# pyxploiter/HandMvNet

Measured on AMD Instinct MI355X. Metric: samples/sec (BxV frames) eval_fps.py, 8-view 256x256; 21-kpt L2 vs reference, higher is better.
Workload: dtype f32; 1 GPU; BASELINE configs[2]: B=32/GPU x V=8 x 256x256, resnet50_paper backbone, d=524, cross_attn x5, GCN decoder; global_batch=32, views=8, frame=256, parallelism=sample-shard x1

## Files before the change

handmvnet_amd/csrc/conv_stream.hip:

```cpp
#include <cstdio>
#include <cstdlib>
#include <type_traits>
#include <utility>

#include "kernels.h"

namespace hmv {

typedef float sf32x16 __attribute__((ext_vector_type(16)));
typedef float sf32x4 __attribute__((ext_vector_type(4)));
typedef _Float16 sf16x8 __attribute__((ext_vector_type(8)));

#define HMV_SGLDS16(gptr, lptr)                                                                             \
    __builtin_amdgcn_global_load_lds((const __attribute__((address_space(1))) void *)(gptr),                \
                                     (__attribute__((address_space(3))) void *)(lptr), 16, 0, 0)

template <int N>
__device__ __forceinline__ void wait_vm() {
    static_assert(N >= 0 && N < 64, "vmcnt is a 6-bit field");
    asm volatile("s_waitcnt vmcnt(%0)" ::"n"(N) : "memory");
}
template <typename F, int... I>
__device__ __forceinline__ void static_for_impl(F &&f, std::integer_sequence<int, I...>) {
    (f(std::integral_constant<int, I>{}), ...);
}
template <int N, typename F>
__device__ __forceinline__ void static_for(F &&f) {
    static_for_impl(static_cast<F &&>(f), std::make_integer_sequence<int, N>{});
}

constexpr int sched_r(int RB, int RS, int j) { return RS ? RS : (j == 0 ? RB : 0); }
constexpr int sched_ops(int NP, int PA, int RB, int RS, int OS, int slot) { return slot < NP ? PA + sched_r(RB, RS, slot) : OS; }
constexpr int sched_after_piece(int NP, int D, int PA, int RB, int RS, int OS, int j) {
    const int T0 = 8, g = T0 * NP + j - D, tq = g / NP, jq = g - tq * NP;
    int n = sched_r(RB, RS, jq);
    for (int s = tq * (NP + 1) + jq + 1; s < T0 * (NP + 1) + j; ++s) n += sched_ops(NP, PA, RB, RS, OS, s % (NP + 1));
    return n;
}
constexpr int sched_after_residual(int NP, int PA, int RB, int RS, int OS) {
    const int T0 = 8, last = RS ? NP - 1 : 0;
    int n = 0;
    for (int s = (T0 - 1) * (NP + 1) + last + 1; s < T0 * (NP + 1) + NP; ++s) n += sched_ops(NP, PA, RB, RS, OS, s % (NP + 1));
    return n;
}
static_assert(sched_after_piece(4, 3, 1, 8, 0, 8, 0) == 10 && sched_after_piece(4, 3, 1, 8, 0, 8, 1) == 18 && sched_after_piece(4, 3, 1, 8, 0, 8, 2) == 18 &&
              sched_after_piece(4, 3, 1, 8, 0, 8, 3) == 10 && sched_after_residual(4, 1, 8, 0, 8) == 23, "the step-0 schedule of four pieces, counted by hand");
static_assert(sched_after_piece(4, 3, 1, 8, 2, 8, 0) == 2 + 3 + 3 + 8 && sched_after_residual(4, 1, 8, 2, 8) == 8 + 4 * 3, "the spread K = 256 schedule");

template <int TM, int TN, int MW, int NW, int NP, int NSLOT, bool HAS_RES, bool SPREAD = false, bool DUAL = false, int N2 = 0>
__global__ __launch_bounds__(64 * MW *NW, (MW * NW) / 4) void conv_stream_f16(const ConvParams p) {
    constexpr int NWV = MW * NW, NT = 64 * NWV;
    constexpr int BM = 32 * TM * MW, BN = 32 * TN * NW;
    constexpr int D = NSLOT - 1;
    constexpr int PA = BM * 8 / NT;
    constexpr int NB2 = N2 / 32;
    constexpr int TM2 = N2 ? (BM / 32) * NB2 / NWV : 0;
    constexpr int K2Q = BN / 16;
    static_assert(N2 == 0 || (N2 % 32 == 0 && TN == 2 && TM2 >= 1 && NWV % NB2 == 0 && (BM / 32) == (NWV / NB2) * TM2),
                  "chain: a wave's 64 output channels are one pixel piece of the second reduction; whole blocks per wave");
    constexpr int RB = HAS_RES ? TM * TN * 2 : 0, OS = TM * TN * 2 + 2 * TM2;
    constexpr int RS = (SPREAD && HAS_RES) ? RB / NP : 0;
    static_assert(!SPREAD || RB % NP == 0, "spread schedule: whole residual DMAs per step");
    constexpr int ZW = TM * TN * 2 * 1024;
    constexpr int NFAKE = (D + NP - 1) / NP;
    static_assert(NT == 512 && BM % 64 == 0 && PA >= 1, "eight waves; whole DMA passes per piece");
    static_assert((NSLOT & (NSLOT - 1)) == 0 && NSLOT >= 2, "a power of two");
    extern __shared__ __attribute__((aligned(16))) char ssm[];
    _Float16 *sA = reinterpret_cast<_Float16 *>(ssm);
    char *zones = ssm + NSLOT * BM * 128;

    const int tid = threadIdx.x, lane = tid & 63;
    const int wave = __builtin_amdgcn_readfirstlane(tid >> 6);
    const int l31 = lane & 31, kh = lane >> 5;
    const int mw = wave / NW, nw = wave - mw * NW;
    const int zi = N2 ? nw * MW + mw : wave;
    static_assert(N2 == 0 || !HAS_RES || ZW == TM * 32 * 128, "chain: a landing zone is the wave's region of the tile image");

    const int nsl = p.ntiles;
    const int loc = (int)blockIdx.x >> 3, per_xcd = 32 / nsl;
    const int slice = loc % nsl, stream = ((int)blockIdx.x & 7) * per_xcd + loc / nsl, nstreams = 8 * per_xcd;
    const int ntl = p.mtiles > stream ? (p.mtiles - stream + nstreams - 1) / nstreams : 0;
    if (ntl == 0) return;
    const int n0 = slice * BN + nw * TN * 32;

    const _Float16 *zero16 = reinterpret_cast<const _Float16 *>(p.zero);
    _Float16 *trash = reinterpret_cast<_Float16 *>(const_cast<float *>(p.zero) + 64 + 4 * lane);
    const _Float16 *Ain = reinterpret_cast<const _Float16 *>(p.in);
    const _Float16 *Rin = reinterpret_cast<const _Float16 *>(p.res);
    _Float16 *Out = reinterpret_cast<_Float16 *>(p.out);

    const int wl31 = (l31 & 0x13) | ((l31 & 4) << 1) | ((l31 & 8) >> 1);
    sf16x8 wreg[TN][NP * 4];
    {
        const _Float16 *wb = reinterpret_cast<const _Float16 *>(p.wgt) + (size_t)(n0 + wl31) * p.ldw + 8 * kh;
#pragma unroll
        for (int b = 0; b < TN; ++b)
#pragma unroll
            for (int Q = 0; Q < NP * 4; ++Q) wreg[b][Q] = *reinterpret_cast<const sf16x8 *>(wb + (size_t)(32 * b) * p.ldw + 16 * Q);
    }
    const int ob2 = N2 ? wave % (N2 ? NB2 : 1) : 0, pg2 = N2 ? wave / (N2 ? NB2 : 1) : 0;
    sf16x8 w2reg[N2 ? K2Q : 1];
    if constexpr (N2 > 0) {
        const _Float16 *wb2 = reinterpret_cast<const _Float16 *>(p.nx_wgt) + (size_t)(32 * ob2 + wl31) * p.nx_ldw + 8 * kh;
#pragma unroll
        for (int Q = 0; Q < K2Q; ++Q) w2reg[Q] = *reinterpret_cast<const sf16x8 *>(wb2 + 16 * Q);
    }
    asm volatile("s_waitcnt vmcnt(0)" ::: "memory");

    const int arow = tid >> 3, kqs = (tid & 7) ^ ((tid >> 4) & 7);
    const int fsw = (l31 >> 1) & 7;

    size_t off2[DUAL ? PA : 1] = {};
    auto issue_A = [&](int G) {
        const int tt = G >= 0 ? G / NP : -1, jj = G >= 0 ? G - tt * NP : 0, slot = G & (NSLOT - 1);
        const int mt = stream + tt * nstreams;
#pragma unroll
        for (int i = 0; i < PA; ++i) {
            const int m = mt * BM + i * 64 + arow;
            const bool ok = tt >= 0 && tt < ntl && m < p.M;
            const _Float16 *src = zero16;
            if constexpr (DUAL) {
                if (jj * 64 == p.ksplit) {
                    const int hw = p.Ho * p.Wo, n = m / hw, rem = m - n * hw, ho = rem / p.Wo, wo = rem - ho * p.Wo;
                    off2[i] = ((size_t)(n * p.H2 + ho * p.stride2) * p.W2 + wo * p.stride2) * p.lda2 + 8 * kqs;
                }
                if (ok && jj * 64 >= p.ksplit) {
                    src = reinterpret_cast<const _Float16 *>(p.in2) + off2[i] + (jj * 64 - p.ksplit);
                } else if (ok) {
                    src = Ain + (size_t)m * p.lda + jj * 64 + 8 * kqs;
                }
// ... 122 lines not shown
                                            (unsigned)((nw * BM + (mw * TM + a) * 32 + l31) * 128 + (((4 * b + 2 * j + kh) ^ fsw) * 16));
                        asm volatile("ds_write_b128 %0, %1" ::"v"(ya), "v"(hv[a][b][j]) : "memory");
                    }
            }
            asm volatile("s_waitcnt lgkmcnt(0)\n\ts_barrier" ::: "memory");
            const __attribute__((address_space(4))) float *bq =
                (const __attribute__((address_space(4))) float *)(p.nx_bias + __builtin_amdgcn_readfirstlane(32 * ob2)) + bz;
            sf32x16 acc2[TM2];
#pragma unroll
            for (int e = 0; e < 16; ++e) {
                const int c = 16 * (e >> 3) + (e & 7);
                const float v0 = bq[c], v1 = bq[c + 8];
                const float v = kh ? v1 : v0;
#pragma unroll
                for (int a = 0; a < TM2; ++a) acc2[a][e] = v;
            }
            const unsigned yr = (unsigned)(size_t)(__attribute__((address_space(3))) char *)yt + (unsigned)((pg2 * TM2 * 32 + l31) * 128);
            constexpr int G = 4 / TM2, NG = K2Q / G;
            static_assert(K2Q % G == 0 && G * TM2 == 4, "four fragment reads per group");
            sf16x8 px[2][G][TM2];
#define HMV_CHAIN_READ_GROUP(g)                                                                                                     \
    _Pragma("unroll") for (int i = 0; i < G; ++i) _Pragma("unroll") for (int a = 0; a < TM2; ++a) {                                \
        const int Q = (g) * G + i;                                                                                                  \
        const unsigned ad = yr + (unsigned)(((Q >> 2) * BM + a * 32) * 128) + (unsigned)((((2 * (Q & 3) + kh) ^ fsw)) * 16);        \
        asm volatile("ds_read_b128 %0, %1" : "=v"(px[(g) & 1][i][a]) : "v"(ad) : "memory");                                         \
    }
            HMV_CHAIN_READ_GROUP(0)
#pragma unroll
            for (int g = 0; g < NG; ++g) {
                sf16x8(&pg)[G][TM2] = px[g & 1];
                if (g + 1 < NG) {
                    HMV_CHAIN_READ_GROUP(g + 1)
                    if constexpr (TM2 == 1) asm volatile("s_waitcnt lgkmcnt(4)" : "+v"(pg[0][0]), "+v"(pg[1][0]), "+v"(pg[2][0]), "+v"(pg[3][0]) :: "memory");
                    else asm volatile("s_waitcnt lgkmcnt(4)" : "+v"(pg[0][0]), "+v"(pg[0][1]), "+v"(pg[1][0]), "+v"(pg[1][1]) :: "memory");
                } else {
                    if constexpr (TM2 == 1) asm volatile("s_waitcnt lgkmcnt(0)" : "+v"(pg[0][0]), "+v"(pg[1][0]), "+v"(pg[2][0]), "+v"(pg[3][0]) :: "memory");
                    else asm volatile("s_waitcnt lgkmcnt(0)" : "+v"(pg[0][0]), "+v"(pg[0][1]), "+v"(pg[1][0]), "+v"(pg[1][1]) :: "memory");
                }
#pragma unroll
                for (int i = 0; i < G; ++i)
#pragma unroll
                    for (int a = 0; a < TM2; ++a) acc2[a] = __builtin_amdgcn_mfma_f32_32x32x16_f16(w2reg[g * G + i], pg[i][a], acc2[a], 0, 0, 0);
            }
#undef HMV_CHAIN_READ_GROUP
            const float lo2 = (p.nx_act == ACT_RELU) ? 0.f : -INFINITY;
            _Float16 *Out2 = reinterpret_cast<_Float16 *>(p.nx_out);
#pragma unroll
            for (int a = 0; a < TM2; ++a) {
                const int m = mt * BM + (pg2 * TM2 + a) * 32 + l31;
                _Float16 *orow = Out2 + (size_t)m * p.nx_ldc + 32 * ob2 + 8 * kh;
#pragma unroll
                for (int j = 0; j < 2; ++j) {
                    const sf16x8 r = {0, 0, 0, 0, 0, 0, 0, 0};
                    sf16x8 h2;
#pragma unroll
                    for (int u = 0; u < 8; ++u) h2[u] = (_Float16)fmaxf(acc2[a][8 * j + u] * p.acc_scale + (float)r[u], lo2);
                    _Float16 *dst = m < p.M ? orow + 16 * j : trash;
                    asm volatile("global_store_dwordx4 %0, %1, off\n\ts_nop 1" ::"v"(dst), "v"(h2) : "memory");
                }
            }
        } else {
#pragma unroll
        for (int a = 0; a < TM; ++a) {
            const int m = mt * BM + (mw * TM + a) * 32 + l31;
            _Float16 *orow = Out + (size_t)m * p.ldc + n0 + 8 * kh;
#pragma unroll
            for (int b = 0; b < TN; ++b)
#pragma unroll
                for (int j = 0; j < 2; ++j) {
                    sf16x8 r = {0, 0, 0, 0, 0, 0, 0, 0};
                    if constexpr (HAS_RES) r = *reinterpret_cast<const sf16x8 *>(z + ((a * TN + b) * 2 + j) * 1024);
                    sf16x8 hv;
#pragma unroll
                    for (int u = 0; u < 8; ++u) hv[u] = (_Float16)fmaxf(acc[a][b][8 * j + u] * p.acc_scale + (float)r[u], lo);
                    _Float16 *dst = m < p.M ? orow + 32 * b + 16 * j : trash;
                    asm volatile("global_store_dwordx4 %0, %1, off\n\ts_nop 1" ::"v"(dst), "v"(hv) : "memory");
                }
        }
        }
    }
    asm volatile("s_waitcnt vmcnt(0) lgkmcnt(0)" ::: "memory");
}

template <int TM, int TN, int MW, int NW, int NP, int NSLOT, bool HAS_RES, bool DUAL = false, bool HALF = false>
__global__ __launch_bounds__(64 * MW *NW, 2) void conv_stream_f32(const ConvParams p) {
    constexpr int NWV = MW * NW, NT = 64 * NWV;
    constexpr int BM = 32 * TM * MW, BN = 32 * TN * NW;
    constexpr int D = NSLOT - 1;
    constexpr int PA = BM * 8 / NT;
    constexpr int RB = HAS_RES ? TM * TN * 4 : 0, OS = TM * TN * 4, RS = 0;
    constexpr int ZW = TM * TN * 4 * 1024;
    constexpr int NFAKE = (D + NP - 1) / NP;
    constexpr int RPP = NT / 8;
    static_assert((NT == 512 || (HALF && NT == 256)) && BM % RPP == 0 && PA >= 1 && (!HALF || (HAS_RES && !DUAL)), "whole DMA passes per piece");
    static_assert((NSLOT & (NSLOT - 1)) == 0 && NSLOT >= 2, "a power of two");
    extern __shared__ __attribute__((aligned(16))) char ssm[];
    float *sA = reinterpret_cast<float *>(ssm);
    char *zones = ssm + NSLOT * BM * 128;

    const int tid = threadIdx.x, lane = tid & 63;
    const int wave = __builtin_amdgcn_readfirstlane(tid >> 6);
    const int l31 = lane & 31, kh = lane >> 5;
    const int mw = wave / NW, nw = wave - mw * NW;
    const int nsl = p.ntiles;
    const int loc = (int)blockIdx.x >> 3, per_xcd = ((int)gridDim.x >> 3) / nsl;
    const int slice = loc % nsl, stream = ((int)blockIdx.x & 7) * per_xcd + loc / nsl, nstreams = 8 * per_xcd;
    const int ntl = p.mtiles > stream ? (p.mtiles - stream + nstreams - 1) / nstreams : 0;
    if (ntl == 0) return;
    const int n0 = slice * BN + nw * TN * 32;

    const float *zero32 = p.zero;
    float *trash = const_cast<float *>(p.zero) + 64 + 4 * lane;
    const float *Ain = reinterpret_cast<const float *>(p.in);
    const float *Rin = reinterpret_cast<const float *>(p.res);
    float *Out = reinterpret_cast<float *>(p.out);

    sf32x4 wreg[TN][NP * 4], bias[TN][4];
    {
        const float *wb = reinterpret_cast<const float *>(p.wgt) + (size_t)(n0 + l31) * p.ldw + 4 * kh;
#pragma unroll
        for (int b = 0; b < TN; ++b) {
#pragma unroll
            for (int Q = 0; Q < NP * 4; ++Q) wreg[b][Q] = *reinterpret_cast<const sf32x4 *>(wb + (size_t)(32 * b) * p.ldw + 8 * Q);
#pragma unroll
            for (int g = 0; g < 4; ++g) bias[b][g] = *reinterpret_cast<const sf32x4 *>(p.bias + n0 + 32 * b + 8 * g + 4 * kh);
        }
    }
    asm volatile("s_waitcnt vmcnt(0)" ::: "memory");

    const int arow = tid >> 3, kqs = (tid & 7) ^ ((tid >> 4) & 7);
    const int fsw = (l31 >> 1) & 7;
    auto issue_A = [&](int G) {
        const int tt = G >= 0 ? G / NP : -1, jj = G >= 0 ? G - tt * NP : 0, slot = G & (NSLOT - 1);
        const int mt = stream + tt * nstreams;
#pragma unroll
        for (int i = 0; i < PA; ++i) {
            const int m = mt * BM + i * RPP + arow;
            const bool ok = tt >= 0 && tt < ntl && m < p.M;
            const float *src = zero32;
            if constexpr (DUAL) {
                if (ok && jj * 32 >= p.ksplit) {
                    const int hw = p.Ho * p.Wo, n = m / hw, rem = m - n * hw, ho = rem / p.Wo, wo = rem - ho * p.Wo;
                    src = reinterpret_cast<const float *>(p.in2) + ((size_t)(n * p.H2 + ho * p.stride2) * p.W2 + wo * p.stride2) * p.lda2 +
                          (jj * 32 - p.ksplit) + 4 * kqs;
                } else if (ok) {
                    src = Ain + (size_t)m * p.lda + jj * 32 + 4 * kqs;
                }
            } else if (ok) {
                src = Ain + (size_t)m * p.lda + jj * 32 + 4 * kqs;
            }
            asm volatile("" : "+v"(src));
            HMV_SGLDS16(src, sA + ((slot * BM + i * RPP + wave * 8) * 32));
        }
    };
    auto issue_R = [&](int tt) {
        if constexpr (HAS_RES) {
            const int mt = stream + tt * nstreams;
            char *z = zones + ((HALF ? 0 : (tt & 1)) * NWV + wave) * ZW;
#pragma unroll
            for (int idx = 0; idx < RB; ++idx) {
                const int a = idx / (4 * TN), b = (idx / 4) % TN, g = idx & 3;
                const int m = mt * BM + (mw * TM + a) * 32 + l31;
                const bool ok = tt >= 0 && tt < ntl && m < p.M;
                const float *src = ok ? Rin + (size_t)m * p.ldr + n0 + 32 * b + 8 * g + 4 * kh : zero32;
                asm volatile("" : "+v"(src));
                HMV_SGLDS16(src, z + idx * 1024);
            }
        }
    };
#pragma unroll
    for (int ft = -NFAKE; ft < 0; ++ft) {
        static_for<NP>([&](auto jc) {
            constexpr int j = decltype(jc)::value;
            issue_A(ft * NP + j + D);
            if constexpr (j == 0) issue_R(HALF ? ft : ft + 1);
        });
#pragma unroll
        for (int i = 0; i < OS; ++i)
            asm volatile("global_store_dwordx4 %0, %1, off\n\ts_nop 1" ::"v"(trash), "v"(sf32x4{0.f, 0.f, 0.f, 0.f}) : "memory");
    }

    const float lo = (p.act == ACT_RELU) ? 0.f : -INFINITY;
    sf32x16 acc[TM][TN];
    for (int tt = 0; tt < ntl; ++tt) {
#pragma unroll
        for (int a = 0; a < TM; ++a)
#pragma unroll
            for (int b = 0; b < TN; ++b)
#pragma unroll
                for (int e = 0; e < 16; ++e) acc[a][b][e] = 0.f;
        static_for<NP>([&](auto jc) {
            constexpr int j = decltype(jc)::value;
            wait_vm<sched_after_piece(NP, D, PA, RB, RS, OS, j)>();
            asm volatile("s_waitcnt lgkmcnt(0)\n\ts_barrier" ::: "memory");
            issue_A(tt * NP + j + D);
            if constexpr (j == 0) issue_R(HALF ? tt : tt + 1);
            const float *pa = sA + ((((tt * NP + j) & (NSLOT - 1)) * BM + mw * TM * 32 + l31) * 32);
#pragma unroll
            for (int q = 0; q < 4; ++q) {
                sf32x4 px[TM];
#pragma unroll
                for (int a = 0; a < TM; ++a) px[a] = *reinterpret_cast<const sf32x4 *>(pa + a * 32 * 32 + (((2 * q + kh) ^ fsw) * 4));
#pragma unroll
                for (int e = 0; e < 4; ++e)
#pragma unroll
                    for (int a = 0; a < TM; ++a)
#pragma unroll
                        for (int b = 0; b < TN; ++b)
                            acc[a][b] = __builtin_amdgcn_mfma_f32_32x32x2f32(wreg[b][4 * j + q][e], px[a][e], acc[a][b], 0, 0, 0);
            }
        });
        if constexpr (HAS_RES) wait_vm<HALF ? (NP - 1) * PA : sched_after_residual(NP, PA, RB, RS, OS)>();
        const int mt = stream + tt * nstreams;
        const char *z = zones + ((HALF ? 0 : (tt & 1)) * NWV + wave) * ZW + lane * 16;
#pragma unroll
        for (int a = 0; a < TM; ++a) {
            const int m = mt * BM + (mw * TM + a) * 32 + l31;
            float *orow = Out + (size_t)m * p.ldc + n0 + 4 * kh;
#pragma unroll
            for (int b = 0; b < TN; ++b)
#pragma unroll
                for (int g = 0; g < 4; ++g) {
                    sf32x4 r = {0.f, 0.f, 0.f, 0.f};
                    if constexpr (HAS_RES) r = *reinterpret_cast<const sf32x4 *>(z + ((a * TN + b) * 4 + g) * 1024);
                    sf32x4 t;
#pragma unroll
                    for (int u = 0; u < 4; ++u) t[u] = fmaxf((acc[a][b][4 * g + u] + bias[b][g][u]) + r[u], lo);
                    float *dst = m < p.M ? orow + 32 * b + 8 * g : trash;
                    asm volatile("global_store_dwordx4 %0, %1, off\n\ts_nop 1" ::"v"(dst), "v"(t) : "memory");
                }
        }
    }
    asm volatile("s_waitcnt vmcnt(0) lgkmcnt(0)" ::: "memory");
}

template <int TM, int TN, int MW, int NW, int NP, int NSLOT, bool HAS_RES, bool SPREAD = false, bool DUAL = false, int N2 = 0>
static hipError_t launch_stream_one(ConvParams p, hipStream_t s) {
    constexpr int BM = 32 * TM * MW, BN = 32 * TN * NW, NWV = MW * NW;
    constexpr size_t lds = (size_t)NSLOT * BM * 128 + (HAS_RES ? (size_t)2 * NWV * TM * TN * 2 * 1024 : (N2 ? (size_t)BM * BN * 2 : 0));
    static_assert(lds <= 160 * 1024, "LDS budget");
    auto kern = conv_stream_f16<TM, TN, MW, NW, NP, NSLOT, HAS_RES, SPREAD, DUAL, N2>;
    if (N2 && (p.Cout != BN || p.nx_cout != N2 || !p.nx_wgt || !p.nx_bias || !p.nx_out)) return hipErrorInvalidValue;
    static DeviceOnce once;
    if (const hipError_t e = once.run([&](int) { return set_max_lds(lds, kern); }); e != hipSuccess) return e;
    p.mtiles = (p.M + BM - 1) / BM;
    p.ntiles = p.Cout / BN;
    hipLaunchKernelGGL(kern, dim3(256), dim3(64 * NWV), lds, s, p);
    return hipGetLastError();
}

static int stream_bn(const ConvParams &p, int *bm = nullptr) {
    int bn = 0, m = 0;
    if (p.in2) {
        if (!p.res && p.Kpad == 128 && p.ksplit == 64 && p.Cout == 256) { bn = 256; m = 128; }
        else if (!p.res && p.Kpad == 384 && p.ksplit == 128 && p.Cout == 512) { bn = 256; m = 64; }
    } else if (p.res) {
        if (p.Kpad == 256 || p.Kpad == 128) { bn = 512; m = 64; }
        else if (p.Kpad == 64) { bn = 256; m = 128; }
    } else {
        if (p.Kpad == 256 && p.Cout == 64) { bn = 64; m = 256; }
        else if (p.Kpad == 512 && p.Cout == 128) { bn = 128; m = 128; }
        else if (p.Kpad == 256 && p.Cout == 128) { bn = 128; m = 128; }
        else if (p.Kpad == 64 && p.Cout == 64) { bn = 64; m = 256; }
    }
    if (bm) *bm = m;
    return bn;
}

static int stream32_shape(const ConvParams &p) {
    if (p.in_f16 || p.out_f16) return 0;
    if (p.in2) return (!p.res && p.Kpad == 128 && p.ksplit == 64 && p.Cout == 256 && p.lda == p.ksplit && p.lda2 % 4 == 0) ? 3 : 0;
    if (p.res) return (!p.res_f16 && (p.Kpad == 64 || p.Kpad == 128 || p.Kpad == 256) && p.Cout % 256 == 0 && 32 % (p.Cout / 256) == 0) ? 1 : 0;
    return (p.Kpad == 256 && p.Cout == 64) ? 2 : ((p.Kpad == 64 && p.Cout == 64) ? 4 : 0);
}
static bool stream32_rule(const ConvParams &p) {
    static const bool no256 = HMV_DEV_ENV("HMV_NO_STREAM32_K256") != nullptr;
    return p.res ? (p.Kpad <= 128 || (!no256 && p.Cout % 128 == 0 && 64 % (p.Cout / 128) == 0)) : true;
}

bool conv_stream_supported(const ConvParams &p, const ConvRoute &route) {
    static const int min_env = HMV_DEV_INT("HMV_STREAM_MIN_TILES", 4);
    if (route.stream == ROUTE_NEVER) return false;
    const bool force = route.stream == ROUTE_FORCE;
    const int min_tiles = force ? 0 : min_env;
    if (stream32_shape(p)) {
        static const bool off32 = HMV_DEV_ENV("HMV_NO_STREAM32") != nullptr;
        if (off32 && !force) return false;
        if (p.R != 1 || p.S != 1 || p.stride != 1 || p.pad_h || p.pad_w || p.up || p.ksl > 1 || p.phases > 1) return false;
        if (p.cwrap || p.x3_plane || p.res_split || p.out_split || p.acc_shift || p.rd_cout || p.scatter || p.rg_out || p.fill) return false;
        if (p.act != ACT_NONE && p.act != ACT_RELU) return false;
        if ((!p.in2 && p.Cin != p.Kpad) || p.K != p.Kpad) return false;
        if ((p.lda ? p.lda : p.Cin) % 4 || (p.ldw ? p.ldw : p.Kpad) % 4 || p.ldc % 4 || (p.res && p.ldr % 4)) return false;
        if (force) return true;
        const int bm32 = (p.res || p.in2) ? 64 : 128, streams32 = p.res ? 256 / (p.Cout / 256) : 256;
        return stream32_rule(p) && (long long)(p.M + bm32 - 1) / bm32 >= (long long)min_tiles * streams32;
    }
    int bm = 0;
    const int bn = stream_bn(p, &bm);
    if (!bn || !p.in_f16 || !p.out_f16 || (p.res && !p.res_f16)) return false;
    if (p.R != 1 || p.S != 1 || p.stride != 1 || p.pad_h || p.pad_w || p.up || p.ksl > 1 || p.phases > 1) return false;
    if (p.in2 && ((p.lda2 & 7) || (p.ksplit & 63) || p.lda != p.ksplit)) return false;
    if (p.cwrap || p.x3_plane || p.res_split || p.out_split || p.acc_shift || p.rd_cout || p.scatter || p.rg_out || p.fill) return false;
    if (p.act != ACT_NONE && p.act != ACT_RELU) return false;
    if ((!p.in2 && p.Cin != p.Kpad) || p.K != p.Kpad || p.Cout % bn != 0 || 32 % (p.Cout / bn) != 0) return false;
    if ((p.lda ? p.lda : p.Cin) % 8 || (p.ldw ? p.ldw : p.Kpad) % 8 || p.ldc % 8 || (p.res && p.ldr % 8)) return false;
    const int streams = 256 / (p.Cout / bn);
    return (long long)(p.M + bm - 1) / bm >= (long long)min_tiles * streams;
}

bool conv_stream_chain_ok(const ConvParams &q, int nx_cout, const ConvRoute &route) {
    static const bool off = HMV_DEV_ENV("HMV_NO_CHAIN") != nullptr;
    if (off || (nx_cout != 64 && nx_cout != 128)) return false;
    ConvParams p = q;
    p.nx_wgt = nullptr;
    if (!p.lda) p.lda = p.Cin;
    if (!p.ldw) p.ldw = p.Kpad;
    if (!p.in_f16 || !p.out_f16 || p.acc_shift || p.Cout != 256 || (p.ldc & 7)) return false;
    if (!(p.in2 ? (!p.res && p.Kpad == 128 && p.ksplit == 64 && nx_cout == 64) : (p.res && p.Kpad == 64))) return false;
    return conv_stream_supported(p, route);
}

template <int TM, int TN, int MW, int NW, int NP, int NSLOT, bool HAS_RES, bool DUAL = false, bool HALF = false>
static hipError_t launch_stream32(ConvParams p, hipStream_t s) {
    constexpr int BM = 32 * TM * MW, BN = 32 * TN * NW;
    constexpr size_t lds = (size_t)NSLOT * BM * 128 + (HAS_RES ? (size_t)(HALF ? 1 : 2) * MW * NW * TM * TN * 4 * 1024 : 0);
    static_assert(lds * (HALF ? 2 : 1) <= 160 * 1024, "LDS budget");
    auto kern = conv_stream_f32<TM, TN, MW, NW, NP, NSLOT, HAS_RES, DUAL, HALF>;
    static DeviceOnce once;
    if (const hipError_t e = once.run([&](int) { return set_max_lds(lds, kern); }); e != hipSuccess) return e;
    p.mtiles = (p.M + BM - 1) / BM;
    p.ntiles = p.Cout / BN;
    hipLaunchKernelGGL(kern, dim3(HALF ? 512 : 256), dim3(64 * MW * NW), lds, s, p);
    return hipGetLastError();
}

hipError_t launch_conv_stream(const ConvParams &p, hipStream_t s, const char **name) {
    if (const int k32 = stream32_shape(p)) {
        if (k32 == 2) { if (name) *name = "conv_stream_f32<128x64,k256>"; return launch_stream32<1, 1, 4, 2, 8, 8, false>(p, s); }
        if (k32 == 4) { if (name) *name = "conv_stream_f32<128x64,k64>"; return launch_stream32<1, 1, 4, 2, 2, 8, false>(p, s); }
        if (k32 == 3) { if (name) *name = "conv_stream_f32<64x256,k128,dual>"; return launch_stream32<2, 1, 1, 8, 4, 8, false, true>(p, s); }
        if (p.Kpad == 256 && p.Cout % 128 == 0 && 64 % (p.Cout / 128) == 0) {
            if (name) *name = "conv_stream_f32<64x128,k256,res>";
            return launch_stream32<2, 1, 1, 4, 8, 4, true, false, true>(p, s);
        }
        if (p.Kpad == 256) { if (name) *name = "conv_stream_f32<64x256,k256,res>"; return launch_stream32<2, 1, 1, 8, 8, 4, true>(p, s); }
        if (p.Kpad == 128) { if (name) *name = "conv_stream_f32<64x256,k128,res>"; return launch_stream32<2, 1, 1, 8, 4, 4, true>(p, s); }
        if (name) *name = "conv_stream_f32<64x256,k64,res>";
        return launch_stream32<2, 1, 1, 8, 2, 4, true>(p, s);
    }
    if (p.nx_wgt) {
        if (p.nx_ldw < p.Cout || (p.nx_ldw & 7) || (p.nx_ldc & 7) || (p.nx_act != ACT_NONE && p.nx_act != ACT_RELU) || p.acc_shift) return hipErrorInvalidValue;
        if (p.in2 && p.Kpad == 128 && p.nx_cout == 64) {
            if (name) *name = "conv_stream_f16<128x256,k128,dual,+1x1:64>";
            return launch_stream_one<2, 2, 2, 4, 2, 4, false, false, true, 64>(p, s);
        }
        if (p.res && p.Kpad == 64 && p.nx_cout == 64) {
            if (name) *name = "conv_stream_f16<128x256,k64,res,+1x1:64>";
            return launch_stream_one<2, 2, 2, 4, 1, 2, true, false, false, 64>(p, s);
        }
        if (p.res && p.Kpad == 64 && p.nx_cout == 128) {
            if (name) *name = "conv_stream_f16<128x256,k64,res,+1x1:128>";
            return launch_stream_one<2, 2, 2, 4, 1, 2, true, false, false, 128>(p, s);
        }
        return hipErrorInvalidValue;
    }
    if (p.in2) {
        if (p.Kpad == 128) {
            if (name) *name = "conv_stream_f16<128x256,k128,dual>";
            return launch_stream_one<2, 2, 2, 4, 2, 8, false, false, true>(p, s);
        }
        if (name) *name = "conv_stream_f16<64x256,k384,dual>";
        return launch_stream_one<2, 1, 1, 8, 6, 8, false, false, true>(p, s);
    }
    if (!p.res) {
        if (p.Kpad == 256 && p.Cout == 64) {
            if (name) *name = "conv_stream_f16<256x64,k256>";
            return launch_stream_one<1, 2, 8, 1, 4, 4, false>(p, s);
        }
        if (p.Kpad == 64 && p.Cout == 64) {
            if (name) *name = "conv_stream_f16<256x64,k64>";
            return launch_stream_one<1, 2, 8, 1, 1, 4, false>(p, s);
        }
        if (p.Kpad == 512) {
            if (name) *name = "conv_stream_f16<128x128,k512>";
            return launch_stream_one<2, 1, 2, 4, 8, 8, false>(p, s);
        }
        if (name) *name = "conv_stream_f16<128x128,k256>";
        return launch_stream_one<1, 2, 4, 2, 4, 8, false>(p, s);
    }
    if (p.Kpad == 256) {
        if (name) *name = "conv_stream_f16<64x512,k256,res>";
        return launch_stream_one<2, 2, 1, 8, 4, 4, true, true>(p, s);
    }
    if (p.Kpad == 128) {
        if (name) *name = "conv_stream_f16<64x512,k128,res>";
        return launch_stream_one<2, 2, 1, 8, 2, 4, true>(p, s);
    }
    if (p.Kpad == 64) {
        if (name) *name = "conv_stream_f16<128x256,k64,res>";
        return launch_stream_one<2, 2, 2, 4, 1, 2, true>(p, s);
    }
    return hipErrorInvalidValue;
}

}
```

handmvnet_amd/csrc/engine.hip:

```cpp
#include <hip/hip_runtime.h>

#include <algorithm>
#include <array>
#include <cmath>
#include <cstdarg>
#include <cstdio>
#include <cstdlib>
#include <cstring>
#include <map>
#include <string>
#include <vector>

#include "../../include/handmv.h"
#include "kernels.h"

using namespace hmv;

namespace {

constexpr int NJ = 21, HEADS = 8, DHEAD = 128, INNER = HEADS * DHEAD;
constexpr int DHEAD_LQ = 256, INNER_LQ = HEADS * DHEAD_LQ;
const int kBlocks[3][4] = {{2, 2, 2, 2}, {3, 4, 6, 3}, {3, 4, 6, 3}};
const int kHrChannels[2][4] = {{40, 80, 160, 320}, {64, 128, 256, 512}};
inline int cpad(int c) { return (c + 3) / 4 * 4; }
// ... 1069 lines not shown
    hmv_engine *h;
    hipStream_t s;
    bool dry;
    int rc = HMV_OK;
    Arena &A;

    float *alloc(size_t n) {
        float *ptr = A.alloc(n);
        if (!dry && h->arena_bytes && A.high > h->arena_bytes && rc == HMV_OK) rc = h->fail(HMV_ERR_STATE, "workspace plan exceeded its reservation");
        return ptr;
    }
    bool defer = false;
    std::vector<float *> deferred;
    void release(float *p) {
        if (defer && p) deferred.push_back(p);
        else A.release(p);
    }
    void fork() {
        defer = true;
        if (dry || rc != HMV_OK) return;
        check(hipEventRecord(h->ev_fork, s), "hipEventRecord");
        check(hipStreamWaitEvent(h->aux, h->ev_fork, 0), "hipStreamWaitEvent");
    }
    void join() {
        if (!dry && rc == HMV_OK) {
            check(hipEventRecord(h->ev_join, h->aux), "hipEventRecord");
            check(hipStreamWaitEvent(s, h->ev_join, 0), "hipStreamWaitEvent");
        }
        defer = false;
        for (float *p : deferred) A.release(p);
        deferred.clear();
    }

    void check(hipError_t e, const char *what) {
        if (e != hipSuccess && rc == HMV_OK) rc = h->fail(HMV_ERR_HIP, "%s: %s", what, hipGetErrorString(e));
    }

    template <class F> void launch(const char *what, F &&f, int n = 1) {
        if (!dry && rc == HMV_OK) { check(f(), what); h->launches += n; }
    }

    const char **kernel_name = nullptr;
    ConvRoute route = conv_rule();

    ConvParams params(const ConvCall &c) const {
        const Layer &L = *c.L;
        ConvParams p{};
        p.in = c.in; p.wgt = L.w; p.bias = L.bias; p.res = c.res; p.out = c.out;
        if (c.ksplit > 1) { p.ksl = c.ksplit; p.kslice = L.Kpad / c.ksplit; p.out_slice = (size_t)c.N * c.Ho * c.Wo * c.ldc; }
        if (c.phases > 1) { p.phases = c.phases; p.phase_stride = c.phase_stride; }
        if (c.dual.in2) {
            p.in2 = c.dual.in2; p.ksplit = c.dual.ksplit; p.H2 = c.dual.H2; p.W2 = c.dual.W2; p.lda2 = c.dual.lda2; p.stride2 = c.dual.stride2;
            p.lda = c.dual.ksplit;
        }
        p.in_f16 = L.f16; p.out_f16 = c.out_f16; p.res_f16 = L.f16 && c.res != nullptr;
        p.N = c.N; p.H = c.H; p.W = c.W; p.Cin = L.Cin;
        p.Ho = c.Ho; p.Wo = c.Wo; p.Cout = L.Cout;
        p.R = L.R; p.S = L.S; p.stride = c.stride; p.pad_h = c.pad_h; p.pad_w = c.pad_w;
        p.K = L.K; p.Kpad = L.Kpad;
        p.M = c.N * c.Ho * c.Wo;
        p.ldc = c.ldc; p.ldr = c.ldr; p.act = c.activation;
        p.rg_out = c.rg_out; p.rg_in = c.rg_in;
        p.scatter = c.scatter; p.osy = c.scatter ? 2 : 1; p.osx = c.scatter ? 2 : 1; p.ooy = c.ooy; p.oox = c.oox;
        p.up = c.up; p.fill = c.fill ? 1 : 0;
        p.tall = L.tall;
        if (L.rd_cout) { p.rd_cout = L.rd_cout; p.pad_w = 0; }
        if (L.plane) {
            p.lda = 2 * L.plane;
            if (L.x3n) p.x3_plane = L.plane;
            else p.cwrap = 2 * L.plane;
            p.acc_shift = L.acc_shift;
            if (c.out_f16) { p.out_split = 1; p.ldc = 2 * c.ldc; p.sat = h->sat; }
            if (c.res) { p.res_split = 1; p.ldr = 2 * c.ldr; }
        }
        if (c.pool_h > 0) { p.pool = 1; p.pool_h = c.pool_h; p.pool_w = c.pool_w; }
        if (const Layer *Lx = c.next) {
            p.nx_wgt = Lx->w; p.nx_bias = Lx->bias; p.nx_out = c.next_out; p.nx_cout = Lx->Cout; p.nx_ldw = Lx->Kpad; p.nx_ldc = Lx->Cout;
            p.nx_act = ACT_RELU;
        }
        return p;
    }

    bool chains_into(const ConvCall &c3, const Block *nb) const {
        if (!h->chain_fuse || !nb || h->cfg.dtype != HMV_F16) return false;
        const Layer &n1 = nb->c1;
        const int outc = c3.L->Cout;
        return n1.f16 && !n1.plane && n1.R == 1 && n1.S == 1 && n1.Cin == outc && n1.K == outc && n1.Kpad == outc && !n1.tall && !n1.rd_cout &&
               conv_stream_chain_ok(params(c3), n1.Cout, route);
    }

    ProfRec *prof_begin(std::string label) {
        if (h->prof_used == h->prof.size()) {
            ProfRec r{};
            check(hipEventCreate(&r.e0), "hipEventCreate");
            check(hipEventCreate(&r.e1), "hipEventCreate");
            h->prof.push_back(r);
        }
        ProfRec *pr = &h->prof[h->prof_used++];
        pr->label = std::move(label);
        check(hipEventRecord(pr->e0, s), "hipEventRecord");
        return pr;
    }
    void prof_end(ProfRec *pr, const char *kernel) {
        if (pr) { pr->name = kernel; check(hipEventRecord(pr->e1, s), "hipEventRecord"); }
    }

    static void conv_cost(const ConvCall &c, const ConvParams &p, double &flops, double &bytes) {
        const Layer &L = *c.L;
        const double kreal = L.Kreal ? (double)L.Kreal : (double)L.K;
        const double cout_real = L.rd_cout ? (double)L.rd_cout : (double)L.Cout;
        const double eb_in = L.f16 ? (L.plane ? 4.0 : 2.0) : 4.0;
        const double eb_out = (L.f16 && c.out_f16) ? (L.plane ? 4.0 : 2.0) : 4.0;
        const double cin_real = L.in_real ? (double)L.in_real : kreal / (double)(L.R * L.S);
        const bool pointwise = L.R == 1 && L.S == 1;
        const double in_px = (pointwise && c.stride > 1) ? (double)p.M : (double)c.N * c.H * c.W;
        const double in_b = in_px * cin_real * eb_in, w_b = (double)L.Cout * kreal * eb_in, out_b = (double)p.M * cout_real * eb_out;
        flops = 2.0 * (double)p.M * (double)L.Cout * kreal;
        if (c.phases > 1) flops *= c.phases;
        if (p.pool)
            bytes = in_b + w_b + (double)c.N * p.pool_h * p.pool_w * cout_real * eb_out;
        else if (c.dual.in2)
            bytes = ((double)p.M * c.dual.ksplit + (double)p.M * (kreal - c.dual.ksplit)) * eb_in + w_b + out_b;
        else if (c.phases > 1)
            bytes = in_b + c.phases * (w_b + out_b);
        else
            bytes = in_b + w_b + out_b + (c.res ? (double)p.M * cout_real * eb_in : 0.0);
        if (const Layer *Lx = c.next) {
            flops += 2.0 * (double)p.M * (double)Lx->Cout * (double)Lx->K;
            bytes += (double)Lx->Cout * (double)Lx->K * eb_in + (double)p.M * (double)Lx->Cout * eb_out;
        }
    }

    void conv(const ConvCall &c) {
        if (dry || rc != HMV_OK) return;
        const Layer &L = *c.L;
        const ConvParams p = params(c);
        const ConvTile tile = conv_pick_tile(p.M, p.Cout, L.plane ? p.K / (L.x3n ? 2 : 3) : p.K, L.f16, c.res != nullptr);
        ProfRec *pr = nullptr;
        if (h->profiling) {
            pr = prof_begin(c.next ? L.label + "+" + c.next->label : (p.pool ? L.label + "+maxpool" : L.label));
            conv_cost(c, p, pr->flops, pr->bytes);
        }
        const char *kname = nullptr;
        check(launch_conv(p, tile, s, &kname, route), L.label.c_str());
        ++h->launches;
        if (kernel_name) *kernel_name = kname;
        prof_end(pr, kname);
    }

    void hr_fuse_up(const HrFuseParams &p, const std::string &label) {
        if (dry || rc != HMV_OK) return;
        ProfRec *pr = nullptr;
        if (h->profiling) {
            pr = prof_begin(label);
            const double eb = p.f16 ? 2.0 : 4.0;
            pr->flops = 0.0;
            pr->bytes = 2.0 * (double)p.N * p.H * p.W * p.C * eb;
            for (int q = 0; q < p.nsrc; ++q) {
                const HrFuseSrc &S = p.src[q];
                pr->flops += 2.0 * (double)p.N * S.H * S.W * S.C * p.C;
                pr->bytes += (double)p.N * S.H * S.W * S.C * eb + (double)S.C * p.C * 4.0;
            }
        }
        check(launch_hr_fuse_up(p, s), label.c_str());
        ++h->launches;
        prof_end(pr, p.f16 ? "hr_fuse_up_f16" : "hr_fuse_up_f32");
    }

    static int splitk_slices(const Layer &L, int rows) {
        static const bool no_splitk = HMV_DEV_ENV("HMV_NO_SPLITK") != nullptr;
// ... 1150 lines not shown
```

Measured before the change: 5976 frames/s.

## Chain the next block's 1x1 conv into the fp32 streamed conv epilogue

Extends the fp32 streaming conv kernel with an N2 template path. The workgroup keeps its 64x256 output tile in LDS after the residual/ReLU epilogue and immediately computes the following bottleneck block's first 1x1 conv (to 64 or 128 channels), split across waves as two K-halves that are summed through LDS. It enables chain fusion for the F32 dtype in the engine. The aim is to remove a separate kernel launch and a global re-read of the 256-channel activation, at the cost of extra barriers, registers for the second weights, and adjusted vmcnt schedules for the waves that store the second output.

```diff
diff --git a/handmvnet_amd/csrc/conv_stream.hip b/handmvnet_amd/csrc/conv_stream.hip
--- a/handmvnet_amd/csrc/conv_stream.hip
+++ b/handmvnet_amd/csrc/conv_stream.hip
@@ -46,6 +46,8 @@
 static_assert(sched_after_piece(4, 3, 1, 8, 0, 8, 0) == 10 && sched_after_piece(4, 3, 1, 8, 0, 8, 1) == 18 && sched_after_piece(4, 3, 1, 8, 0, 8, 2) == 18 &&
               sched_after_piece(4, 3, 1, 8, 0, 8, 3) == 10 && sched_after_residual(4, 1, 8, 0, 8) == 23, "the step-0 schedule of four pieces, counted by hand");
 static_assert(sched_after_piece(4, 3, 1, 8, 2, 8, 0) == 2 + 3 + 3 + 8 && sched_after_residual(4, 1, 8, 2, 8) == 8 + 4 * 3, "the spread K = 256 schedule");
+static_assert(sched_after_piece(2, 3, 1, 8, 0, 16, 0) == 16 + (1 + 8) + 1 + 16 && sched_after_piece(2, 3, 1, 8, 0, 16, 1) == 8 + 1 + 16 + (1 + 8) &&
+              sched_after_residual(2, 1, 8, 0, 16) == 1 + 16 + (1 + 8) + 1, "the chained fp32 K = 64 schedule, counted by hand");
 
 template <int TM, int TN, int MW, int NW, int NP, int NSLOT, bool HAS_RES, bool SPREAD = false, bool DUAL = false, int N2 = 0>
 __global__ __launch_bounds__(64 * MW *NW, (MW * NW) / 4) void conv_stream_f16(const ConvParams p) {
@@ -334,13 +336,18 @@
     asm volatile("s_waitcnt vmcnt(0) lgkmcnt(0)" ::: "memory");
 }
 
-template <int TM, int TN, int MW, int NW, int NP, int NSLOT, bool HAS_RES, bool DUAL = false, bool HALF = false>
+template <int TM, int TN, int MW, int NW, int NP, int NSLOT, bool HAS_RES, bool DUAL = false, bool HALF = false, int N2 = 0>
 __global__ __launch_bounds__(64 * MW *NW, 2) void conv_stream_f32(const ConvParams p) {
     constexpr int NWV = MW * NW, NT = 64 * NWV;
     constexpr int BM = 32 * TM * MW, BN = 32 * TN * NW;
     constexpr int D = NSLOT - 1;
     constexpr int PA = BM * 8 / NT;
     constexpr int RB = HAS_RES ? TM * TN * 4 : 0, OS = TM * TN * 4, RS = 0;
+    constexpr int NB2 = N2 / 32;
+    constexpr int TM2 = N2 ? (BM / 32) * NB2 / 4 : 0;
+    constexpr int OS2 = 4 * TM2, OSF = OS + OS2;
+    static_assert(N2 == 0 || ((N2 == 64 || N2 == 128) && TM == 2 && TN == 1 && MW == 1 && NW == 8 && !HALF && HAS_RES != DUAL),
+                  "chain: the workgroup owns 64 pixels x 256 channels, one 32-channel block (= one piece of the second reduction) per wave");
     constexpr int ZW = TM * TN * 4 * 1024;
     constexpr int NFAKE = (D + NP - 1) / NP;
     constexpr int RPP = NT / 8;
@@ -368,6 +375,14 @@
     float *Out = reinterpret_cast<float *>(p.out);
 
     sf32x4 wreg[TN][NP * 4], bias[TN][4];
+    const bool fin = N2 && wave >= 4;
+    const int ob2 = N2 ? (wave & 3) % (N2 ? NB2 : 1) : 0, pg2 = N2 ? (wave & 3) / (N2 ? NB2 : 1) : 0;
+    sf32x4 w2reg[N2 ? 16 : 1];
+    if constexpr (N2 > 0) {
+        const float *wb2 = reinterpret_cast<const float *>(p.nx_wgt) + (size_t)(32 * ob2 + l31) * p.nx_ldw + (fin ? 128 : 0) + 4 * kh;
+#pragma unroll
+        for (int Q = 0; Q < 16; ++Q) w2reg[Q] = *reinterpret_cast<const sf32x4 *>(wb2 + 8 * Q);
+    }
     {
         const float *wb = reinterpret_cast<const float *>(p.wgt) + (size_t)(n0 + l31) * p.ldw + 4 * kh;
 #pragma unroll
@@ -430,7 +445,22 @@
 #pragma unroll
         for (int i = 0; i < OS; ++i)
             asm volatile("global_store_dwordx4 %0, %1, off\n\ts_nop 1" ::"v"(trash), "v"(sf32x4{0.f, 0.f, 0.f, 0.f}) : "memory");
-    }
+        if constexpr (N2 > 0) {
+            if (fin) {
+#pragma unroll
+                for (int i = 0; i < OS2; ++i)
+                    asm volatile("global_store_dwordx4 %0, %1, off\n\ts_nop 1" ::"v"(trash), "v"(sf32x4{0.f, 0.f, 0.f, 0.f}) : "memory");
+            }
+        }
+    }
+    auto wait_counted = [&](auto na, auto nf) {
+        if constexpr (N2 > 0) {
+            if (fin) wait_vm<decltype(nf)::value>();
+            else wait_vm<decltype(na)::value>();
+        } else {
+            wait_vm<decltype(na)::value>();
+        }
+    };
 
     const float lo = (p.act == ACT_RELU) ? 0.f : -INFINITY;
     sf32x16 acc[TM][TN];
@@ -443,7 +473,8 @@
                 for (int e = 0; e < 16; ++e) acc[a][b][e] = 0.f;
         static_for<NP>([&](auto jc) {
             constexpr int j = decltype(jc)::value;
-            wait_vm<sched_after_piece(NP, D, PA, RB, RS, OS, j)>();
+            wait_counted(std::integral_constant<int, sched_after_piece(NP, D, PA, RB, RS, OS, j)>{},
+                         std::integral_constant<int, sched_after_piece(NP, D, PA, RB, RS, OSF, j)>{});
             asm volatile("s_waitcnt lgkmcnt(0)\n\ts_barrier" ::: "memory");
             issue_A(tt * NP + j + D);
             if constexpr (j == 0) issue_R(HALF ? tt : tt + 1);
@@ -462,9 +493,121 @@
                             acc[a][b] = __builtin_amdgcn_mfma_f32_32x32x2f32(wreg[b][4 * j + q][e], px[a][e], acc[a][b], 0, 0, 0);
             }
         });
-        if constexpr (HAS_RES) wait_vm<HALF ? (NP - 1) * PA : sched_after_residual(NP, PA, RB, RS, OS)>();
+        if constexpr (HAS_RES)
+            wait_counted(std::integral_constant<int, HALF ? (NP - 1) * PA : sched_after_residual(NP, PA, RB, RS, OS)>{},
+                         std::integral_constant<int, sched_after_residual(NP, PA, RB, RS, OSF)>{});
         const int mt = stream + tt * nstreams;
         const char *z = zones + ((HALF ? 0 : (tt & 1)) * NWV + wave) * ZW + lane * 16;
+        if constexpr (N2 > 0) {
+            char *yt = HAS_RES ? zones + (tt & 1) * NWV * ZW : zones;
+            const unsigned yt3 = (unsigned)(size_t)(__attribute__((address_space(3))) char *)yt;
+            sf32x4 rr[TM][4], tv[TM][4];
+            if constexpr (HAS_RES) {
+#pragma unroll
+                for (int a = 0; a < TM; ++a)
+#pragma unroll
+                    for (int g = 0; g < 4; ++g) rr[a][g] = *reinterpret_cast<const sf32x4 *>(z + (a * 4 + g) * 1024);
+            }
+#pragma unroll
+            for (int a = 0; a < TM; ++a) {
+                const int m = mt * BM + a * 32 + l31;
+                float *orow = Out + (size_t)m * p.ldc + n0 + 4 * kh;
+#pragma unroll
+                for (int g = 0; g < 4; ++g) {
+                    sf32x4 r = {0.f, 0.f, 0.f, 0.f};
+                    if constexpr (HAS_RES) r = rr[a][g];
+#pragma unroll
+                    for (int u = 0; u < 4; ++u) tv[a][g][u] = fmaxf((acc[a][0][4 * g + u] + bias[0][g][u]) + r[u], lo);
+                    float *dst = m < p.M ? orow + 8 * g : trash;
+                    asm volatile("global_store_dwordx4 %0, %1, off\n\ts_nop 1" ::"v"(dst), "v"(tv[a][g]) : "memory");
+                    if constexpr (!HAS_RES) {
+                        const unsigned ya = yt3 + (unsigned)((nw * BM + a * 32 + l31) * 128 + (((2 * g + kh) ^ fsw) * 16));
+                        asm volatile("ds_write_b128 %0, %1" ::"v"(ya), "v"(tv[a][g]) : "memory");
+                    }
+                }
+            }
+            if constexpr (HAS_RES) {
+#pragma unroll
+                for (int a = 0; a < TM; ++a)
+#pragma unroll
+                    for (int g = 0; g < 4; ++g) {
+                        const unsigned ya = yt3 + (unsigned)((nw * BM + a * 32 + l31) * 128 + (((2 * g + kh) ^ fsw) * 16));
+                        asm volatile("ds_write_b128 %0, %1" ::"v"(ya), "v"(tv[a][g]) : "memory");
+                    }
+            }
+            asm volatile("s_waitcnt lgkmcnt(0)\n\ts_barrier" ::: "memory");
+            sf32x16 acc2[TM2];
+            const float *yr = reinterpret_cast<const float *>(yt) + ((fin ? 4 : 0) * BM + pg2 * TM2 * 32 + l31) * 32;
+            auto half_gemm = [&]() {
+#pragma unroll
+                for (int jj = 0; jj < 4; ++jj)
+#pragma unroll
+                    for (int q = 0; q < 4; ++q) {
+                        sf32x4 px[TM2];
+#pragma unroll
+                        for (int a = 0; a < TM2; ++a) px[a] = *reinterpret_cast<const sf32x4 *>(yr + (jj * BM + a * 32) * 32 + (((2 * q + kh) ^ fsw) * 4));
+#pragma unroll
+                        for (int e = 0; e < 4; ++e)
+#pragma unroll
+                            for (int a = 0; a < TM2; ++a)
+                                acc2[a] = __builtin_amdgcn_mfma_f32_32x32x2f32(w2reg[4 * jj + q][e], px[a][e], acc2[a], 0, 0, 0);
+                    }
+            };
+            if (!fin) {
+#pragma unroll
+                for (int a = 0; a < TM2; ++a)
+#pragma unroll
+                    for (int e = 0; e < 16; ++e) acc2[a][e] = 0.f;
+                half_gemm();
+            }
+            asm volatile("s_waitcnt lgkmcnt(0)\n\ts_barrier" ::: "memory");
+            if (!fin) {
+                const unsigned hand3 = yt3 + (unsigned)((wave & 3) * TM2 * 4096 + lane * 16);
+#pragma unroll
+                for (int a = 0; a < TM2; ++a)
+#pragma unroll
+                    for (int g = 0; g < 4; ++g) {
+                        const sf32x4 v = {acc2[a][4 * g], acc2[a][4 * g + 1], acc2[a][4 * g + 2], acc2[a][4 * g + 3]};
+                        asm volatile("ds_write_b128 %0, %1" ::"v"(hand3 + (unsigned)(a * 4096 + g * 1024)), "v"(v) : "memory");
+                    }
+            }
+            asm volatile("s_waitcnt lgkmcnt(0)\n\ts_barrier" ::: "memory");
+            if (fin) {
+                const char *hand = yt + (wave & 3) * TM2 * 4096 + lane * 16;
+#pragma unroll
+                for (int a = 0; a < TM2; ++a)
+#pragma unroll
+                    for (int g = 0; g < 4; ++g) {
+                        const sf32x4 v = *reinterpret_cast<const sf32x4 *>(hand + a * 4096 + g * 1024);
+#pragma unroll
+                        for (int u = 0; u < 4; ++u) acc2[a][4 * g + u] = v[u];
+                    }
+                half_gemm();
+                int bz;
+                asm volatile("s_mov_b32 %0, 0" : "=s"(bz));
+                const __attribute__((address_space(4))) float *bq =
+                    (const __attribute__((address_space(4))) float *)(p.nx_bias + __builtin_amdgcn_readfirstlane(32 * ob2)) + bz;
+                const float lo2 = (p.nx_act == ACT_RELU) ? 0.f : -INFINITY;
+                float *Out2 = reinterpret_cast<float *>(p.nx_out);
+#pragma unroll
+                for (int a = 0; a < TM2; ++a) {
+                    const int m = mt * BM + (pg2 * TM2 + a) * 32 + l31;
+                    float *orow = Out2 + (size_t)m * p.nx_ldc + 32 * ob2 + 4 * kh;
+#pragma unroll
+                    for (int g = 0; g < 4; ++g) {
+                        const sf32x4 r = {0.f, 0.f, 0.f, 0.f};
+                        sf32x4 t;
+#pragma unroll
+                        for (int u = 0; u < 4; ++u) {
+                            const float b0 = bq[8 * g + u], b1 = bq[8 * g + 4 + u];
+                            t[u] = fmaxf((acc2[a][4 * g + u] + (kh ? b1 : b0)) + r[u], lo2);
+                        }
+                        float *dst = m < p.M ? orow + 8 * g : trash;
+                        asm volatile("global_store_dwordx4 %0, %1, off\n\ts_nop 1" ::"v"(dst), "v"(t) : "memory");
+                    }
+                }
+            }
+        } else {
 #pragma unroll
         for (int a = 0; a < TM; ++a) {
             const int m = mt * BM + (mw * TM + a) * 32 + l31;
@@ -481,6 +624,7 @@
                     float *dst = m < p.M ? orow + 32 * b + 8 * g : trash;
                     asm volatile("global_store_dwordx4 %0, %1, off\n\ts_nop 1" ::"v"(dst), "v"(t) : "memory");
                 }
+        }
         }
     }
     asm volatile("s_waitcnt vmcnt(0) lgkmcnt(0)" ::: "memory");
@@ -567,17 +711,23 @@
     p.nx_wgt = nullptr;
     if (!p.lda) p.lda = p.Cin;
     if (!p.ldw) p.ldw = p.Kpad;
+    if (!p.in_f16) {
+        if (p.out_f16 || p.res_f16 || p.acc_shift || p.Cout != 256 || (p.ldc & 3)) return false;
+        if (!(p.in2 ? (stream32_shape(p) == 3 && nx_cout == 64) : (p.res && p.Kpad == 64 && stream32_shape(p) == 1))) return false;
+        return conv_stream_supported(p, route);
+    }
     if (!p.in_f16 || !p.out_f16 || p.acc_shift || p.Cout != 256 || (p.ldc & 7)) return false;
     if (!(p.in2 ? (!p.res && p.Kpad == 128 && p.ksplit == 64 && nx_cout == 64) : (p.res && p.Kpad == 64))) return false;
     return conv_stream_supported(p, route);
 }
 
-template <int TM, int TN, int MW, int NW, int NP, int NSLOT, bool HAS_RES, bool DUAL = false, bool HALF = false>
+template <int TM, int TN, int MW, int NW, int NP, int NSLOT, bool HAS_RES, bool DUAL = false, bool HALF = false, int N2 = 0>
 static hipError_t launch_stream32(ConvParams p, hipStream_t s) {
     constexpr int BM = 32 * TM * MW, BN = 32 * TN * NW;
-    constexpr size_t lds = (size_t)NSLOT * BM * 128 + (HAS_RES ? (size_t)(HALF ? 1 : 2) * MW * NW * TM * TN * 4 * 1024 : 0);
+    constexpr size_t lds = (size_t)NSLOT * BM * 128 + (HAS_RES ? (size_t)(HALF ? 1 : 2) * MW * NW * TM * TN * 4 * 1024 : (N2 ? (size_t)BM * BN * 4 : 0));
     static_assert(lds * (HALF ? 2 : 1) <= 160 * 1024, "LDS budget");
-    auto kern = conv_stream_f32<TM, TN, MW, NW, NP, NSLOT, HAS_RES, DUAL, HALF>;
+    auto kern = conv_stream_f32<TM, TN, MW, NW, NP, NSLOT, HAS_RES, DUAL, HALF, N2>;
+    if (N2 && (p.Cout != BN || p.nx_cout != N2 || !p.nx_wgt || !p.nx_bias || !p.nx_out)) return hipErrorInvalidValue;
     static DeviceOnce once;
     if (const hipError_t e = once.run([&](int) { return set_max_lds(lds, kern); }); e != hipSuccess) return e;
     p.mtiles = (p.M + BM - 1) / BM;
@@ -588,6 +738,23 @@
 
 hipError_t launch_conv_stream(const ConvParams &p, hipStream_t s, const char **name) {
     if (const int k32 = stream32_shape(p)) {
+        if (p.nx_wgt) {
+            if (p.nx_ldw < p.Cout || (p.nx_ldw & 3) || (p.nx_ldc & 3) || (p.nx_act != ACT_NONE && p.nx_act != ACT_RELU) || p.acc_shift || p.Cout != 256)
+                return hipErrorInvalidValue;
+            if (k32 == 3 && p.nx_cout == 64) {
+                if (name) *name = "conv_stream_f32<64x256,k128,dual,+1x1:64>";
+                return launch_stream32<2, 1, 1, 8, 4, 8, false, true, false, 64>(p, s);
+            }
+            if (k32 == 1 && p.Kpad == 64 && p.nx_cout == 64) {
+                if (name) *name = "conv_stream_f32<64x256,k64,res,+1x1:64>";
+                return launch_stream32<2, 1, 1, 8, 2, 4, true, false, false, 64>(p, s);
+            }
+            if (k32 == 1 && p.Kpad == 64 && p.nx_cout == 128) {
+                if (name) *name = "conv_stream_f32<64x256,k64,res,+1x1:128>";
+                return launch_stream32<2, 1, 1, 8, 2, 4, true, false, false, 128>(p, s);
+            }
+            return hipErrorInvalidValue;
+        }
         if (k32 == 2) { if (name) *name = "conv_stream_f32<128x64,k256>"; return launch_stream32<1, 1, 4, 2, 8, 8, false>(p, s); }
         if (k32 == 4) { if (name) *name = "conv_stream_f32<128x64,k64>"; return launch_stream32<1, 1, 4, 2, 2, 8, false>(p, s); }
         if (k32 == 3) { if (name) *name = "conv_stream_f32<64x256,k128,dual>"; return launch_stream32<2, 1, 1, 8, 4, 8, false, true>(p, s); }
diff --git a/handmvnet_amd/csrc/engine.hip b/handmvnet_amd/csrc/engine.hip
--- a/handmvnet_amd/csrc/engine.hip
+++ b/handmvnet_amd/csrc/engine.hip
@@ -1175,10 +1175,10 @@
     }
 
     bool chains_into(const ConvCall &c3, const Block *nb) const {
-        if (!h->chain_fuse || !nb || h->cfg.dtype != HMV_F16) return false;
+        if (!h->chain_fuse || !nb || (h->cfg.dtype != HMV_F16 && h->cfg.dtype != HMV_F32)) return false;
         const Layer &n1 = nb->c1;
         const int outc = c3.L->Cout;
-        return n1.f16 && !n1.plane && n1.R == 1 && n1.S == 1 && n1.Cin == outc && n1.K == outc && n1.Kpad == outc && !n1.tall && !n1.rd_cout &&
+        return n1.f16 == (h->cfg.dtype == HMV_F16) && !n1.plane && n1.R == 1 && n1.S == 1 && n1.Cin == outc && n1.K == outc && n1.Kpad == outc && !n1.tall && !n1.rd_cout &&
                conv_stream_chain_ok(params(c3), n1.Cout, route);
     }
 
```

Result: no change. 6001 frames/s (median of 6 runs) (+0.4%).
